# drdh/Homophily-MARL

Measured on NVIDIA B200. Metric: agent-steps/sec (step+obs, device-timed), higher is better.
Workload: dtype u8

## Files before the change

homophily_marl_b200/csrc/ssd_b200.cu:

```cuda
#include <cuda_runtime.h>
#include <stdint.h>
#include <stdlib.h>
#include <string.h>
#include <math.h>
#include <new>
#include <mutex>

#include "ssd_b200.h"

namespace {

constexpr int kWarps = 4;
constexpr int kMinBlocks = 8;
using ColourLuts = uint32_t[kWarps][16];
constexpr uint16_t kNoPoint = 0xFFFF;
constexpr int kMaxDevices = 64;

enum { MODE_STEP = 0, MODE_RESET = 1, MODE_RENDER = 2 };

#ifdef SSD_BOUNDS_CHECK
__device__ unsigned long long g_oob_count = 0;
#define SSD_CHECK(cond) do { if (!(cond)) atomicAdd(&g_oob_count, 1ull); } while (0)
#else
#define SSD_CHECK(cond) do { } while (0)
#endif

struct MapDev {
    uint8_t  base_grid[SSD_MAX_CELLS];
    uint16_t apple_pts[SSD_MAX_CELLS + 4];
    uint16_t waste_pts[SSD_MAX_CELLS + 4];
    uint16_t spawn_pts[SSD_MAX_SPAWN];
    uint32_t thr_apple[SSD_MAX_CELLS + 1];
    uint32_t thr_waste[SSD_MAX_CELLS + 1];
};

struct GeoVals {
    int kind, H, W, V, G, GS, N, RP, PS, AS, LPn, nw8M, nw8T, pitchM, pitchT, PMS;
    int off_map[4];
    int direct, padF, padB;
    uint32_t maskM8;
    int RS4, AS4;
};
__host__ __device__ constexpr int cround_up(int v, int m) { return (v + m - 1) / m * m; }
__host__ __device__ constexpr GeoVals make_geo(int kind, int H, int W, int V) {
    GeoVals g{};
    g.kind = kind; g.H = H; g.W = W; g.V = V; g.G = H * W; g.GS = cround_up(H * W, 16);
    g.N = 2 * V + 1; g.RP = cround_up(g.N, 4); g.PS = g.N * g.RP; g.AS = cround_up(3 * g.PS, 16);
    g.LPn = cround_up(V, 8); g.nw8M = (W + 7) / 8; g.nw8T = (H + 7) / 8;
    g.maskM8 = (W & 7) ? (1u << (4 * (W & 7))) - 1u : 0xffffffffu;
    int wm = (g.LPn + W + V + 7) / 8; if (wm < g.LPn / 8 + g.nw8M) wm = g.LPn / 8 + g.nw8M; if ((wm & 1) == 0) ++wm;
    int wt = (g.LPn + H + V + 7) / 8; if (wt < g.LPn / 8 + g.nw8T) wt = g.LPn / 8 + g.nw8T; if ((wt & 1) == 0) ++wt;
    g.pitchM = 4 * wm; g.pitchT = 4 * wt;
    const int szM = cround_up((H + 2 * V) * g.pitchM, 16) + 16, szT = cround_up((W + 2 * V) * g.pitchT, 16) + 16;
    g.off_map[0] = 16; g.off_map[1] = 16; g.off_map[2] = 16 + szT; g.off_map[3] = 16 + szT;
    g.PMS = szT + szM + 32;
    g.direct = g.RP <= 16;
    g.padF = g.direct ? cround_up(V * W + 48, 16) : 16;
    g.padB = g.direct ? cround_up(V * W + 32, 16) : 32;
    if (g.direct) g.PMS = 0;
    g.RS4 = cround_up((g.N + 1) / 2, 4); g.AS4 = cround_up(g.N * g.RS4, 16);
    return g;
}

struct KParams {
    GeoVals geo;
    int B, n;
    int env0, env1;
    int pdl;
    int NA;
    int agents_uniform;
    int episode_limit, fire_cost, hit_penalty, beam_len, n_actions;
    int n_apple, n_waste, n_spawn, n_apple4, n_waste2;
    int random_spawn, spawn_rot;
    int base_apples, base_waste;
    uint32_t invN20, invW20, invMW20;
    uint32_t seed_lo, seed_hi, gid_base;
    uint32_t thr_harvest[4];
    uint32_t lut[16];
    uint32_t lut8[6];
    const MapDev* map;
    uint8_t* grid; uint32_t* agent; int32_t* ep_ret; int32_t* t; uint32_t* tick; uint32_t* counts;
    const uint8_t* actions; const uint8_t* mask;
    int8_t* reward; uint8_t* clean; uint16_t* apple_cnt; uint8_t* done; uint8_t* obs; uint8_t* state_rgb;
    const uint32_t* d_prio; const uint32_t* d_uapple; const uint32_t* d_uwaste; const uint32_t* d_wkey;
    const uint32_t* d_spawnkey; const uint8_t* d_rot;
    int tag_timeout;
    int state_idx4;
};

template <class D>
struct GeoAccess {
    __device__ __forceinline__ int kind() const { return v().kind; }
    __device__ __forceinline__ int H() const { return v().H; }
    __device__ __forceinline__ int W() const { return v().W; }
    __device__ __forceinline__ int V() const { return v().V; }
    __device__ __forceinline__ int G() const { return v().G; }
    __device__ __forceinline__ int GS() const { return v().GS; }
    __device__ __forceinline__ int N() const { return v().N; }
    __device__ __forceinline__ int RP() const { return v().RP; }
    __device__ __forceinline__ int PS() const { return v().PS; }
    __device__ __forceinline__ int AS() const { return v().AS; }
    __device__ __forceinline__ int RS4() const { return v().RS4; }
    __device__ __forceinline__ int AS4() const { return v().AS4; }
    __device__ __forceinline__ int LPn() const { return v().LPn; }
    __device__ __forceinline__ int nw8M() const { return v().nw8M; }
    __device__ __forceinline__ int nw8T() const { return v().nw8T; }
    __device__ __forceinline__ int pitchM() const { return v().pitchM; }
    __device__ __forceinline__ int pitchT() const { return v().pitchT; }
    __device__ __forceinline__ int PMS() const { return v().PMS; }
    __device__ __forceinline__ bool direct() const { return v().direct != 0; }
    __device__ __forceinline__ int padF() const { return v().padF; }
    __device__ __forceinline__ int padB() const { return v().padB; }
    __device__ __forceinline__ uint32_t maskM8() const { return v().maskM8; }
private:
    __device__ __forceinline__ decltype(auto) v() const { return static_cast<const D*>(this)->vals(); }
};

template <int KIND_, int H_, int W_, int V_>
struct GeoS : GeoAccess<GeoS<KIND_, H_, W_, V_>> {
    static constexpr GeoVals v = make_geo(KIND_, H_, W_, V_);
    __device__ __forceinline__ explicit GeoS(const KParams&) {}
    __device__ __forceinline__ static constexpr GeoVals vals() { return v; }
    __device__ __forceinline__ int off_map(int o) const {
        constexpr int o0 = v.off_map[0], o1 = v.off_map[1], o2 = v.off_map[2], o3 = v.off_map[3];
        return o == 0 ? o0 : (o == 1 ? o1 : (o == 2 ? o2 : o3));
    }
    __device__ __forceinline__ int divW(int x) const { return (int)((unsigned)x / (unsigned)v.W); }
    __device__ __forceinline__ int divN(int x) const { return (int)((unsigned)x / (unsigned)v.N); }
    __device__ __forceinline__ int divMW(int x) const { return (int)((unsigned)x / (unsigned)v.nw8M); }
};

struct GeoD : GeoAccess<GeoD> {
    const KParams& p;
    __device__ __forceinline__ explicit GeoD(const KParams& p_) : p(p_) {}
    __device__ __forceinline__ const GeoVals& vals() const { return p.geo; }
    __device__ __forceinline__ int off_map(int o) const { return p.geo.off_map[o]; }
    __device__ __forceinline__ int divW(int x) const { return (int)(((uint32_t)x * p.invW20) >> 20); }
    __device__ __forceinline__ int divN(int x) const { return (int)(((uint32_t)x * p.invN20) >> 20); }
    __device__ __forceinline__ int divMW(int x) const { return (int)(((uint32_t)x * p.invMW20) >> 20); }
};

__device__ __forceinline__ uint4 philox4x32_10(uint32_t c0, uint32_t c1, uint32_t c2, uint32_t c3,
                                               uint32_t k0, uint32_t k1) {
#pragma unroll
    for (int r = 0; r < 10; ++r) {
        const uint32_t hi0 = __umulhi(0xD2511F53u, c0), lo0 = 0xD2511F53u * c0;
        const uint32_t hi1 = __umulhi(0xCD9E8D57u, c2), lo1 = 0xCD9E8D57u * c2;
        const uint32_t n0 = hi1 ^ c1 ^ k0, n2 = hi0 ^ c3 ^ k1;
        c0 = n0; c1 = lo1; c2 = n2; c3 = lo0;
        k0 += 0x9E3779B9u; k1 += 0xBB67AE85u;
    }
    return make_uint4(c0, c1, c2, c3);
}
__device__ __forceinline__ uint32_t pick(const uint4& v, int i) {
    return i == 0 ? v.x : (i == 1 ? v.y : (i == 2 ? v.z : v.w));
}
struct Warp {
    int lane;
    __device__ __forceinline__ explicit Warp(int lane_) : lane(lane_) {}
    __device__ __forceinline__ unsigned ballot(bool pred) const { return __ballot_sync(0xffffffffu, pred); }
    template <typename T> __device__ __forceinline__ T shfl(T v, int src) const { return __shfl_sync(0xffffffffu, v, src); }
    template <typename T> __device__ __forceinline__ T rmin(T v) const { return __reduce_min_sync(0xffffffffu, v); }
    template <typename T> __device__ __forceinline__ T rmax(T v) const { return __reduce_max_sync(0xffffffffu, v); }
    template <typename T> __device__ __forceinline__ T radd(T v) const { return __reduce_add_sync(0xffffffffu, v); }
    __device__ __forceinline__ unsigned ror(unsigned v) const { return __reduce_or_sync(0xffffffffu, v); }
    __device__ __forceinline__ void sync() const { __syncwarp(); }
};

__device__ __forceinline__ unsigned equal_lanes(const Warp& w, int v, int n) {
    unsigned m = 0;
    for (int j = 0; j < n; ++j) m |= (unsigned)(w.shfl(v, j) == v) << j;
    return m;
}
__device__ __forceinline__ bool surely_distinct(const Warp& w, int v, bool in, unsigned who) {
    const int cnt = __popc(who);
    const unsigned f0 = w.ror(in ? 1u << (v & 31) : 0u);
    if (__popc(f0) == cnt) return true;
    const unsigned f1 = w.ror(in ? 1u << ((v >> 5) & 31) : 0u);
    return __popc(f1) == cnt;
}

template <typename F>
__device__ __forceinline__ void warp_for(int n, int lane, F f) {
    int i = lane;
    if (i < n) f(i);
    for (i += 32; i < n; i += 32) f(i);
}
__device__ __forceinline__ uint32_t philox_word(const KParams& p, uint32_t gid, uint32_t tick, uint32_t stream, uint32_t idx) {
    const uint4 r = philox4x32_10(gid, tick, stream, idx >> 2, p.seed_lo, p.seed_hi);
    return pick(r, idx & 3);
}

__device__ __forceinline__ int agent_colour_index(int i) {
    const int v = i % 10 + 1;
    return 6 + (v == 10 ? 1 : v);
}

template <class GEO>
__device__ __forceinline__ void update_moves(const Warp& w, const GEO& g, const KParams& p, const uint8_t* __restrict__ sg, int lane, bool is_agent,
                                             int act, int& pos, int& ori, int env, uint32_t gid, uint32_t tick) {
    if (act == 5) ori = (0x0132 >> (4 * ori)) & 3;
    else if (act == 6) ori = (0x1023 >> (4 * ori)) & 3;
    const bool mover = is_agent && act <= 4;
    int prop = pos;
    if (mover && act < 4) {
        constexpr uint32_t kDr = (1u) | (1u << 2) | (0u << 4) | (2u << 6) | (1u << 8) | (1u << 10) | (2u << 12) | (0u << 14) |
                                 (0u << 16) | (2u << 18) | (1u << 20) | (1u << 22) | (2u << 24) | (0u << 26) | (1u << 28) | (1u << 30);
        constexpr uint32_t kDc = (2u) | (0u << 2) | (1u << 4) | (1u << 6) | (0u << 8) | (2u << 10) | (1u << 12) | (1u << 14) |
                                 (1u << 16) | (1u << 18) | (0u << 20) | (2u << 22) | (1u << 24) | (1u << 26) | (2u << 28) | (0u << 30);
        const int f = 2 * (ori * 4 + act);
        const int dr = (int)((kDr >> f) & 3u) - 1, dc = (int)((kDc >> f) & 3u) - 1;
        const int q = pos + dr * g.W() + dc;
        SSD_CHECK(q >= 0 && q < g.G());
        prop = sg[q] == SSD_CELL_WALL ? pos : q;
    }
    unsigned in_moves = w.ballot(mover);
    if (in_moves == 0) return;
    int mv = prop;

    unsigned pending = 0;
    if (!surely_distinct(w, prop, mover, in_moves)) {
        const unsigned grp = equal_lanes(w, mover ? prop : -1000 - lane, p.n);
        pending = w.ballot(mover && __popc(grp) >= 2);
    }
    if (pending) {
        uint32_t prio = 0;
        if (mover) prio = p.d_prio ? p.d_prio[(size_t)env * p.n + lane] : philox_word(p, gid, tick, 0, (uint32_t)lane);
        while (pending) {
            const int cell = w.rmin(((pending >> lane) & 1u) ? prop : 0x7fffffff);
            const bool in_cont = mover && prop == cell;
            const unsigned cont = w.ballot(in_cont);
            const unsigned occm = w.ballot(pos == cell);
            bool free_cell = true;
            if (occm) {
                const int occ = 31 - __clz(occm);
                const int mv_occ = w.shfl(mv, occ);
                const bool occ_moves = (in_moves >> occ) & 1u;
                const bool c1 = (cont >> occ) & 1u;
                const bool c2 = !occ_moves || mv_occ == cell;
                const unsigned swp = w.ballot(in_cont && mv_occ == pos);
// ... 608 lines not shown
            d[0] = (uint8_t)rgb; d[g.PS()] = (uint8_t)(rgb >> 8); d[2 * g.PS()] = (uint8_t)(rgb >> 16);
        }
    }
}

template <int MODE, class GEO, bool TAG, bool IDX>
__global__ void __launch_bounds__(kWarps * 32, kMinBlocks) ssd_kernel(const __grid_constant__ KParams p) {
    const GEO g(p);
    extern __shared__ __align__(16) uint8_t smem[];
    __shared__ ColourLuts lut_all;
    const int warp = threadIdx.x >> 5;
    const Warp w(threadIdx.x & 31);
    const int lane = w.lane;
    uint32_t* lut_s = lut_all[warp];
    uint8_t* tile = smem + (size_t)warp * (g.padF() + g.GS() + g.padB() + g.PMS());
    uint8_t* sg = tile + g.padF();
    uint8_t* pmap = sg + g.GS() + g.padB();
    const bool is_agent = lane < p.n;
    const int env = p.env0 + blockIdx.x * kWarps + warp;
    if (env >= p.env1) return;
    auto prologue = [&]() {
        if (lane < 16) lut_s[lane] = p.lut[lane];
        if (p.obs) {
            if (g.direct()) {
                for (int i = lane; i < (g.padF() >> 4); i += 32) reinterpret_cast<uint4*>(tile)[i] = make_uint4(0, 0, 0, 0);
                for (int i = lane; i < (g.padB() >> 4); i += 32) reinterpret_cast<uint4*>(sg + g.GS())[i] = make_uint4(0, 0, 0, 0);
            } else fill_outside(w, g, p, pmap, lane);
        }
    };
    if (p.pdl) {
        prologue();
        asm volatile("griddepcontrol.wait;" ::: "memory");
    }
    {
        if (MODE == MODE_RESET && p.mask && __ldcg(p.mask + env) == 0) return;
        const uint32_t gid = p.gid_base + (uint32_t)env;
        const uint32_t tick = __ldcg(p.tick + env);
        const int t_prev = MODE == MODE_STEP ? __ldcg(p.t + env) : 0;
        const uint32_t cnt = MODE == MODE_STEP ? __ldcg(p.counts + env) : 0u;
        int act = (MODE == MODE_STEP && is_agent) ? (int)__ldcg(p.actions + (size_t)env * p.n + lane) : 255;
        int pos = -1 - lane, ori = 0, ep_ret = 0;
        uint32_t a_rec = 0;
        if (MODE != MODE_RESET && is_agent) {
            a_rec = __ldcg(p.agent + (size_t)env * p.NA + lane);
            ep_ret = __ldcg(p.ep_ret + (size_t)env * p.NA + lane);
        }
        const int n16 = g.GS() >> 4;
        {
            const uint4* src = MODE == MODE_RESET ? reinterpret_cast<const uint4*>(p.map->base_grid)
                                                  : reinterpret_cast<const uint4*>(p.grid + (size_t)env * g.GS());
            uint4 g0 = make_uint4(0, 0, 0, 0);
            if (lane < n16) g0 = __ldcg(src + lane);
            if (!p.pdl) prologue();
            if (lane < n16) reinterpret_cast<uint4*>(sg)[lane] = g0;
            for (int i = lane + 32; i < n16; i += 32) reinterpret_cast<uint4*>(sg)[i] = __ldcg(src + i);
        }
        bool live = is_agent;
        int timer = 0, home = 0;
        if (MODE != MODE_RESET && is_agent) {
            pos = (int)(a_rec & 0xff) * g.W() + (int)((a_rec >> 8) & 0xff);
            ori = (int)((a_rec >> 16) & 3);
            if (TAG) {
                timer = (int)(a_rec >> 24);
                home = pos;
                if (timer) { live = false; pos = -1 - lane; act = 255; }
            }
        }
        w.sync();

        int apples = (int)(cnt & 0xffffu), waste = (int)(cnt >> 16);
        unsigned same = 1u << lane;
        if (MODE == MODE_RENDER) same = equal_lanes(w, pos, p.n);
        if (MODE == MODE_STEP) {
            int reward = 0, clean_num = 0;
            bool tagged = false;
            update_moves(w, g, p, sg, lane, live, act, pos, ori, env, gid, tick);
            same = surely_distinct(w, pos, live, w.ballot(live)) ? (1u << lane) : equal_lanes(w, pos, p.n);
            const int here = live ? sg[pos] : 0;
            const bool first = live && lane == __ffs(same) - 1;
            const unsigned ate = w.ballot(first && here == SSD_CELL_APPLE);
            w.sync();
            if (first) {
                if (here == SSD_CELL_APPLE) { reward += 1; sg[pos] = kOcc | SSD_CELL_EMPTY; }
                else sg[pos] = (uint8_t)(kOcc | here);
            }
            apples -= __popc(ate);
            w.sync();
            beams<TAG>(w, g, p, sg, lane, live, act, pos, ori, reward, clean_num, waste, tagged);
            unsigned gone = 0;
            if (TAG) {
                gone = w.ballot(tagged);
                if (gone) {
                    if (live && lane == __ffs(same) - 1 && (same & ~gone) == 0) sg[pos] &= 0x7f;
                    w.sync();
                    if (tagged) { home = pos; pos = -1 - lane; live = false; }
                }
            }
            spawn(w, g, p, sg, lane, env, gid, tick, apples, waste);
            if (TAG) {
                const bool back = timer == 1;
                timer = tagged ? p.tag_timeout : (timer ? timer - 1 : 0);
                const unsigned who = w.ballot(back);
                if (who) {
                    place_agents<true>(w, g, p, sg, lane, env, gid, tick, who, pos);
                    if (back) { ori = spawn_orientation(p, env, gid, tick, lane); live = true; sg[pos] |= kOcc; }
                    w.sync();
                }
                if (gone | who) same = equal_lanes(w, pos, p.n);
            }
            const int t = t_prev + 1;
            if (is_agent) {
                p.reward[(size_t)env * p.n + lane] = (int8_t)reward;
                p.clean[(size_t)env * p.n + lane] = (uint8_t)clean_num;
                ep_ret += reward;
            }
            if (lane == 0) {
                p.apple_cnt[env] = (uint16_t)apples;
                p.done[env] = t >= p.episode_limit;
                p.t[env] = t;
                p.tick[env] = tick + 1;
                p.counts[env] = (uint32_t)apples | ((uint32_t)waste << 16);
            }
        } else if (MODE == MODE_RESET) {
            place_agents<false>(w, g, p, sg, lane, env, gid, tick, ~0u, pos);
            if (is_agent) ori = spawn_orientation(p, env, gid, tick, lane);
            if (is_agent) sg[pos] |= kOcc;
            w.sync();
            apples = p.base_apples; waste = p.base_waste;
            spawn(w, g, p, sg, lane, env, gid, tick, apples, waste);
            ep_ret = 0;
            if (lane == 0) { p.t[env] = 0; p.tick[env] = tick + 1; p.counts[env] = (uint32_t)apples | ((uint32_t)waste << 16); }
        }

        if (p.pdl) asm volatile("griddepcontrol.launch_dependents;" ::: "memory");
        if (MODE != MODE_RENDER) {
            if (live && lane == __ffs(same) - 1) sg[pos] &= 0x7f;
            w.sync();
            uint4* dst = reinterpret_cast<uint4*>(p.grid + (size_t)env * g.GS());
            warp_for(g.GS() >> 4, lane, [&](int i) { dst[i] = reinterpret_cast<const uint4*>(sg)[i]; });
            if (is_agent) {
                const int cell = (TAG && !live) ? home : pos;
                const int r = g.divW(cell);
                p.agent[(size_t)env * p.NA + lane] = (uint32_t)r | ((uint32_t)(cell - r * g.W()) << 8) | ((uint32_t)ori << 16)
                                                     | (TAG ? (uint32_t)timer << 24 : 0u);
                p.ep_ret[(size_t)env * p.NA + lane] = ep_ret;
            }
        }
        if (p.obs || p.state_rgb) {
            w.sync();
            if (IDX) { if (live && lane == 31 - __clz(same)) sg[pos] = (uint8_t)(p.agents_uniform ? 7 : agent_colour_index(lane)); }
            else if (live) sg[pos] = 7;
            w.sync();
            const unsigned outm = TAG ? w.ballot(is_agent && !live) : 0u;
            render<IDX>(w, g, p, sg, pmap, lut_s, lane, is_agent, live, pos, ori, env, same, outm);
        }
    }
}

__global__ void incentive_kernel(const long long* __restrict__ a_inc, const float* __restrict__ reward, long long rows, int n,
                                 float incentive, float cost, float ratio, float T, int recip,
                                 float* __restrict__ r_env, float* __restrict__ r_inc, float* __restrict__ sgn) {
    const long long idx = (long long)blockIdx.x * blockDim.x + threadIdx.x;
    if (idx >= rows * n) return;
    const long long row = idx / n;
    const int k = (int)(idx - row * n);
    const long long* a = a_inc + row * n * n;
    int give = 0, rp = 0, rn = 0;
    for (int j = 0; j < n; ++j) {
        if (j == k) continue;
        give += a[k * n + j] != 0;
        const long long v = a[j * n + k];
        rp += v == 1; rn += v == 2;
    }
    const float rv = (float)(rp - rn), r = reward[idx];
    const float e = __fadd_rn(r, __fmul_rn(__fmul_rn(rv, ratio), incentive));
    const float c = __fsub_rn(r, __fmul_rn(__fmul_rn((float)give, cost), incentive));
    if (recip) { const float inv = __fdiv_rn(1.0f, T); r_env[idx] = __fmul_rn(e, inv); r_inc[idx] = __fmul_rn(c, inv); }
    else { r_env[idx] = __fdiv_rn(e, T); r_inc[idx] = __fdiv_rn(c, T); }
    if (sgn) sgn[idx] = rv > 0.f ? 1.f : (rv < 0.f ? -1.f : 0.f);
}

struct ExpandParams {
    const uint8_t* in;
    float* out;
    int rows, cols, row_stride, block_stride;
    uint32_t lut[16];
};
__global__ void __launch_bounds__(256) expand_index4_kernel(const __grid_constant__ ExpandParams p) {
    const uint8_t* __restrict__ in = p.in + (size_t)blockIdx.x * p.block_stride;
    const int NN = p.rows * p.cols;
    float* __restrict__ out = p.out + (size_t)blockIdx.x * 3 * NN;
    for (int q = threadIdx.x; q < NN; q += blockDim.x) {
        const int y = q / p.cols, x = q - y * p.cols;
        const uint32_t rgb = p.lut[(__ldg(in + y * p.row_stride + (x >> 1)) >> (4 * (x & 1))) & 15u];
        out[q] = (float)(rgb & 0xffu) * (1.0f / 256.0f);
        out[NN + q] = (float)((rgb >> 8) & 0xffu) * (1.0f / 256.0f);
        out[2 * NN + q] = (float)((rgb >> 16) & 0xffu) * (1.0f / 256.0f);
    }
}

thread_local int g_last_cuda_error = 0;

inline int cuda_fail(cudaError_t e) { g_last_cuda_error = (int)e; return SSD_ERR_CUDA; }
#define SSD_CUDA(x) do { cudaError_t e_ = (x); if (e_ != cudaSuccess) return cuda_fail(e_); } while (0)

inline int round_up(int v, int m) { return (v + m - 1) / m * m; }

struct DeviceGuard {
    int prev = -1;
    bool switched = false;
    cudaError_t err = cudaSuccess;
    explicit DeviceGuard(int dev) {
        err = cudaGetDevice(&prev);
        if (err == cudaSuccess && prev != dev) { err = cudaSetDevice(dev); switched = err == cudaSuccess; }
    }
    ~DeviceGuard() { if (switched) cudaSetDevice(prev); }
};

uint32_t magic20(int d, int max_x) {
    uint32_t m = (uint32_t)(((1u << 20) + d - 1) / d);
    for (int x = 0; x <= max_x; ++x)
        if ((int)(((uint64_t)x * m) >> 20) != x / d) return 0;
    return m;
}

ssd_obs_layout obs_layout(const KParams& k, int32_t format) {
    const GeoVals& g = k.geo;
    if (format == SSD_OBS_INDEX4) return { format, g.RS4, 0, g.AS4, k.n * g.AS4 };
    return { format, g.RP, g.PS, g.AS, k.n * g.AS };
}

ssd_state_layout state_layout(const KParams& k, int32_t format) {
    const GeoVals& g = k.geo;
    if (format == SSD_OBS_INDEX4) return { format, 4 * g.nw8M, 0, 4 * round_up(g.H * g.nw8M, 4) };
    return { format, g.W, g.G, 3 * g.G };
}

}

struct ssd_handle {
    KParams kp;
    MapDev* d_map;
    int device;
    size_t smem_bytes;
    mutable int64_t launches;
    int force_generic;
    int pdl;
    int obs_format;
    int state_format;
};

static int fill_common(const ssd_handle* h, const ssd_state* st, const ssd_draws* d, KParams& k) {
    if (!h || !st || !st->grid || !st->agent || !st->ep_ret || !st->t || !st->tick || !st->counts) return SSD_ERR_INVALID;
    k = h->kp;
    k.env0 = 0; k.env1 = k.B;
    k.state_idx4 = h->state_format == SSD_OBS_INDEX4;
    k.grid = st->grid; k.agent = st->agent; k.ep_ret = st->ep_ret; k.t = st->t; k.tick = st->tick; k.counts = st->counts;
    if (d) {
        if ((d->u_waste == nullptr) != (d->wkey == nullptr)) return SSD_ERR_INVALID;
        k.d_prio = d->prio; k.d_uapple = d->u_apple; k.d_uwaste = d->u_waste; k.d_wkey = d->wkey;
        k.d_spawnkey = d->spawn_key; k.d_rot = d->rot;
    }
    return SSD_OK;
}

template <int MODE, class GEO, bool TAG, bool IDX>
static int launch_kernel(ssd_handle* h, const KParams& k, void* stream) {
    DeviceGuard guard(h->device);
    SSD_CUDA(guard.err);
    {
        static std::mutex mu;
        static int high_water[kMaxDevices] = {};
        std::lock_guard<std::mutex> lock(mu);
        const int dev = h->device;
        if (dev < 0 || dev >= kMaxDevices) return SSD_ERR_INVALID;
        if ((int)h->smem_bytes > high_water[dev]) {
            SSD_CUDA(cudaFuncSetAttribute(ssd_kernel<MODE, GEO, TAG, IDX>, cudaFuncAttributeMaxDynamicSharedMemorySize, (int)h->smem_bytes));
            high_water[dev] = (int)h->smem_bytes;
        }
    }
    const int grid = (k.env1 - k.env0 + kWarps - 1) / kWarps;
    if (grid <= 0) return SSD_OK;

    if (k.pdl) {
        cudaLaunchConfig_t cfg = {};
        cfg.gridDim = dim3((unsigned)grid); cfg.blockDim = dim3(kWarps * 32); cfg.dynamicSmemBytes = h->smem_bytes;
        cfg.stream = (cudaStream_t)stream;
        cudaLaunchAttribute attr[1];
        attr[0].id = cudaLaunchAttributeProgrammaticStreamSerialization;
        attr[0].val.programmaticStreamSerializationAllowed = 1;
        cfg.attrs = attr; cfg.numAttrs = 1;
        SSD_CUDA(cudaLaunchKernelEx(&cfg, ssd_kernel<MODE, GEO, TAG, IDX>, k));
    } else {
        ssd_kernel<MODE, GEO, TAG, IDX><<<grid, kWarps * 32, h->smem_bytes, (cudaStream_t)stream>>>(k);
    }
    ++h->launches;
    SSD_CUDA(cudaGetLastError());
    return SSD_OK;
}

constexpr int kPdlMaxEnvs = 2048;

template <int MODE, class GEO>
static int launch_geo(ssd_handle* h, const KParams& k_in, void* stream) {
    KParams k = k_in;
    k.pdl = h->pdl && (k.env1 - k.env0) <= kPdlMaxEnvs;
    const bool idx = h->obs_format == SSD_OBS_INDEX4;
    if constexpr (MODE != MODE_RESET) {
        if (k.tag_timeout != 0)
            return idx ? launch_kernel<MODE, GEO, true, true>(h, k, stream) : launch_kernel<MODE, GEO, true, false>(h, k, stream);
    }
    return idx ? launch_kernel<MODE, GEO, false, true>(h, k, stream) : launch_kernel<MODE, GEO, false, false>(h, k, stream);
}

template <int MODE>
static int launch(ssd_handle* h, const KParams& k, void* stream) {
    const GeoVals& v = k.geo;
    if (!h->force_generic) {
        if (v.kind == SSD_KIND_HARVEST && v.H == 9 && v.W == 38 && v.V == 15) return launch_geo<MODE, GeoS<SSD_KIND_HARVEST, 9, 38, 15>>(h, k, stream);
        if (v.kind == SSD_KIND_HARVEST && v.H == 9 && v.W == 38 && v.V == 7) return launch_geo<MODE, GeoS<SSD_KIND_HARVEST, 9, 38, 7>>(h, k, stream);
        if (v.kind == SSD_KIND_CLEANUP && v.H == 25 && v.W == 18 && v.V == 7) return launch_geo<MODE, GeoS<SSD_KIND_CLEANUP, 25, 18, 7>>(h, k, stream);
        if (v.kind == SSD_KIND_CLEANUP && v.H == 48 && v.W == 18 && v.V == 7) return launch_geo<MODE, GeoS<SSD_KIND_CLEANUP, 48, 18, 7>>(h, k, stream);
        if (v.kind == SSD_KIND_CLEANUP && v.H == 10 && v.W == 10 && v.V == 7) return launch_geo<MODE, GeoS<SSD_KIND_CLEANUP, 10, 10, 7>>(h, k, stream);
    }
    return launch_geo<MODE, GeoD>(h, k, stream);
}

extern "C" {

int ssd_abi_version(void) { return SSD_B200_ABI_VERSION; }

const char* ssd_error_string(int code) {
    switch (code) {
        case SSD_OK: return "ok";
        case SSD_ERR_INVALID: return "invalid argument or unsupported geometry";
        case SSD_ERR_CUDA: return "CUDA runtime error";
        case SSD_ERR_SPAWN: return "There are not enough spawn points! Check your map?";
        case SSD_ERR_MAP: return "map must be wall-enclosed and use the reference alphabet";
        default: return "unknown error";
    }
}

int ssd_last_cuda_error(void) { return g_last_cuda_error; }

uint32_t ssd_prob_to_threshold(double p) {
    if (!(p > 0.0)) return 0u;
    const double t = ceil(p * 4294967296.0);
    return t >= 4294967295.0 ? 0xFFFFFFFFu : (uint32_t)t;
}

int ssd_create(const ssd_config* cfg, ssd_handle** out) {
    if (!cfg || !out || !cfg->ascii_map) return SSD_ERR_INVALID;
    *out = nullptr;
    const int H = cfg->height, W = cfg->width, G = H * W, n = cfg->n_agents, V = cfg->view;
    if (cfg->kind != SSD_KIND_CLEANUP && cfg->kind != SSD_KIND_HARVEST) return SSD_ERR_INVALID;
    if (H < 3 || W < 3 || H > 255 || W > 255 || G > SSD_MAX_CELLS) return SSD_ERR_INVALID;
    if (n < 1 || n > SSD_MAX_AGENTS || V < 1 || V > 31 || cfg->n_envs < 1) return SSD_ERR_INVALID;
    if (cfg->beam_len < 0 || cfg->episode_limit < 1 || cfg->spawn_rotation > 3) return SSD_ERR_INVALID;
    if (abs(cfg->fire_cost) + n * abs(cfg->hit_penalty) + 1 > 127) return SSD_ERR_INVALID;
    if (cfg->tag_timeout < 0 || cfg->tag_timeout > 255) return SSD_ERR_INVALID;

    MapDev* hm = new (std::nothrow) MapDev;
    if (!hm) return SSD_ERR_INVALID;
    memset(hm, 0, sizeof(MapDev));
    int na = 0, nw = 0, ns = 0;
    for (int c = 0; c < G; ++c) {
        const char ch = cfg->ascii_map[c];
        const int r = c / W, col = c % W;
        const bool border = r == 0 || col == 0 || r == H - 1 || col == W - 1;
        if (border && ch != '@') { delete hm; return SSD_ERR_MAP; }
        uint8_t code = SSD_CELL_EMPTY;
        switch (ch) {
            case '@': code = SSD_CELL_WALL; break;
            case ' ': break;
            case 'P': if (ns < SSD_MAX_SPAWN) hm->spawn_pts[ns] = (uint16_t)c; ++ns; break;
            case 'A': if (cfg->kind == SSD_KIND_HARVEST) { code = SSD_CELL_APPLE; hm->apple_pts[na++] = (uint16_t)c; } break;
            case 'B': if (cfg->kind == SSD_KIND_CLEANUP) hm->apple_pts[na++] = (uint16_t)c; break;
            case 'H': if (cfg->kind == SSD_KIND_CLEANUP) { code = SSD_CELL_WASTE; hm->waste_pts[nw++] = (uint16_t)c; } break;
            case 'R': if (cfg->kind == SSD_KIND_CLEANUP) code = SSD_CELL_RIVER; break;
            case 'S': if (cfg->kind == SSD_KIND_CLEANUP) code = SSD_CELL_STREAM; break;
            default: delete hm; return SSD_ERR_MAP;
        }
        hm->base_grid[c] = code;
    }
    if (ns < n) { delete hm; return SSD_ERR_SPAWN; }
    if (ns > SSD_MAX_SPAWN) { delete hm; return SSD_ERR_INVALID; }
    for (int k = na; k < round_up(na, 4) + 4 && k < SSD_MAX_CELLS + 4; ++k) hm->apple_pts[k] = kNoPoint;
    for (int k = nw; k < round_up(nw, 2) + 2 && k < SSD_MAX_CELLS + 4; ++k) hm->waste_pts[k] = kNoPoint;
    if (cfg->kind == SSD_KIND_CLEANUP) {
        if (cfg->n_waste_lut != (uint32_t)nw + 1 || !cfg->thr_apple || !cfg->thr_waste) { delete hm; return SSD_ERR_INVALID; }
        memcpy(hm->thr_apple, cfg->thr_apple, sizeof(uint32_t) * (nw + 1));
        memcpy(hm->thr_waste, cfg->thr_waste, sizeof(uint32_t) * (nw + 1));
    }

    ssd_handle* h = new (std::nothrow) ssd_handle;
    if (!h) { delete hm; return SSD_ERR_INVALID; }
    memset(h, 0, sizeof(*h));
    KParams& k = h->kp;
    k.geo = make_geo(cfg->kind, H, W, V);
    const GeoVals& gv = k.geo;
    k.B = cfg->n_envs; k.n = n; k.NA = round_up(n, 4);
    k.episode_limit = cfg->episode_limit; k.fire_cost = cfg->fire_cost; k.hit_penalty = cfg->hit_penalty;
    k.tag_timeout = cfg->tag_timeout;
    k.beam_len = cfg->beam_len; k.n_actions = cfg->kind == SSD_KIND_CLEANUP ? 9 : 8;
    k.n_apple = na; k.n_waste = nw; k.n_spawn = ns; k.n_apple4 = (na + 3) / 4; k.n_waste2 = (nw + 1) / 2;
    k.base_apples = 0; k.base_waste = 0;
    for (int c = 0; c < G; ++c) { k.base_apples += hm->base_grid[c] == SSD_CELL_APPLE; k.base_waste += hm->base_grid[c] == SSD_CELL_WASTE; }
    k.random_spawn = cfg->random_spawn_point != 0; k.spawn_rot = cfg->spawn_rotation < 0 ? -1 : cfg->spawn_rotation;
    k.invN20 = magic20(gv.N, SSD_MAX_AGENTS * gv.N + 64); k.invW20 = magic20(W, G + 1);
    k.seed_lo = (uint32_t)cfg->seed; k.seed_hi = (uint32_t)(cfg->seed >> 32); k.gid_base = cfg->env_gid_base;
    for (int i = 0; i < 4; ++i) k.thr_harvest[i] = cfg->thr_harvest[i];
    for (int i = 0; i < 16; ++i)
        k.lut[i] = (uint32_t)cfg->color_lut[i][0] | ((uint32_t)cfg->color_lut[i][1] << 8) | ((uint32_t)cfg->color_lut[i][2] << 16);
    k.agents_uniform = 1;
    for (int i = 8; i < 16; ++i) if (k.lut[i] != k.lut[7]) k.agents_uniform = 0;
    for (int ch = 0; ch < 3; ++ch) {
        uint32_t lo = 0, hi = 0;
        for (int i = 0; i < 4; ++i) { lo |= (uint32_t)cfg->color_lut[i][ch] << (8 * i); hi |= (uint32_t)cfg->color_lut[4 + i][ch] << (8 * i); }
        k.lut8[2 * ch] = lo; k.lut8[2 * ch + 1] = hi;
    }
    if (k.invN20 == 0 || k.invW20 == 0 || k.n_apple4 > 32 * 16) { delete hm; delete h; return SSD_ERR_INVALID; }

    k.invMW20 = magic20(gv.nw8M, H * gv.nw8M + 32);
    if (k.invMW20 == 0 || gv.PMS >= 60000) { delete hm; delete h; return SSD_ERR_INVALID; }
    h->smem_bytes = (size_t)kWarps * (gv.padF + gv.GS + gv.padB + gv.PMS);
    { const char* e = getenv("SSD_B200_GENERIC"); h->force_generic = e && e[0] == '1'; }
    { const char* e = getenv("SSD_B200_PDL"); h->pdl = !(e && e[0] == '0'); }
    h->device = cfg->device;

    DeviceGuard guard(cfg->device);
    cudaError_t e = guard.err;
    if (e == cudaSuccess) {
        int optin = 0;
        e = cudaDeviceGetAttribute(&optin, cudaDevAttrMaxSharedMemoryPerBlockOptin, cfg->device);
        if (e == cudaSuccess && h->smem_bytes + sizeof(ColourLuts) > (size_t)optin) { delete hm; delete h; return SSD_ERR_INVALID; }
    }
    if (e == cudaSuccess) e = cudaMalloc(&h->d_map, sizeof(MapDev));
    if (e == cudaSuccess) e = cudaMemcpy(h->d_map, hm, sizeof(MapDev), cudaMemcpyHostToDevice);
    delete hm;
    if (e != cudaSuccess) {
        if (h->d_map) cudaFree(h->d_map);
        delete h;
        return cuda_fail(e);
    }
    k.map = h->d_map;
    *out = h;
    return SSD_OK;
}

int ssd_destroy(ssd_handle* h) {
    if (!h) return SSD_ERR_INVALID;
    DeviceGuard guard(h->device);
    cudaFree(h->d_map);
    delete h;
    return SSD_OK;
}

int ssd_get_layout(const ssd_handle* h, ssd_layout* o) {
    if (!h || !o) return SSD_ERR_INVALID;
    const KParams& k = h->kp;
    const GeoVals& g = k.geo;
    o->n_actions = k.n_actions; o->n_cells = g.G; o->obs_n = g.N; o->grid_stride = g.GS; o->agent_stride = k.NA;
    o->obs_plane_stride = g.PS; o->obs_agent_stride = g.AS; o->obs_env_stride = obs_layout(k, SSD_OBS_RGB).env_stride;
    o->n_apple_pts = k.n_apple; o->n_waste_pts = k.n_waste; o->n_spawn_pts = k.n_spawn; o->obs_row_stride = g.RP;
    return SSD_OK;
}

int ssd_get_obs_layout(const ssd_handle* h, int32_t format, ssd_obs_layout* o) {
    if (!h || !o || (format != SSD_OBS_RGB && format != SSD_OBS_INDEX4)) return SSD_ERR_INVALID;
    *o = obs_layout(h->kp, format);
    return SSD_OK;
}

int ssd_set_obs_format(ssd_handle* h, int32_t format) {
    if (!h || (format != SSD_OBS_RGB && format != SSD_OBS_INDEX4)) return SSD_ERR_INVALID;
    h->obs_format = format;
    return SSD_OK;
}

int ssd_get_state_layout(const ssd_handle* h, int32_t format, ssd_state_layout* o) {
    if (!h || !o || (format != SSD_OBS_RGB && format != SSD_OBS_INDEX4)) return SSD_ERR_INVALID;
    *o = state_layout(h->kp, format);
    return SSD_OK;
}

int ssd_set_state_format(ssd_handle* h, int32_t format) {
    if (!h || (format != SSD_OBS_RGB && format != SSD_OBS_INDEX4)) return SSD_ERR_INVALID;
    h->state_format = format;
    return SSD_OK;
}

int ssd_reset(ssd_handle* h, const ssd_state* st, const uint8_t* mask, const ssd_draws* draws, uint8_t* obs, void* stream) {
    KParams k;
    const int rc = fill_common(h, st, draws, k);
    if (rc) return rc;
    k.mask = mask; k.obs = obs;
    return launch<MODE_RESET>(h, k, stream);
}

int ssd_step(ssd_handle* h, const ssd_state* st, const uint8_t* actions, const ssd_draws* draws,
             const ssd_step_out* out, void* stream) {
    return ssd_step_range(h, st, actions, draws, out, 0, h ? h->kp.B : 0, stream);
}

int ssd_step_range(ssd_handle* h, const ssd_state* st, const uint8_t* actions, const ssd_draws* draws,
                   const ssd_step_out* out, int32_t env_begin, int32_t env_count, void* stream) {
    KParams k;
    const int rc = fill_common(h, st, draws, k);
    if (rc) return rc;
    if (!actions || !out || !out->reward || !out->clean || !out->apple_cnt || !out->done) return SSD_ERR_INVALID;
    if (env_begin < 0 || env_count < 0 || (int64_t)env_begin + env_count > k.B) return SSD_ERR_INVALID;
    k.env0 = env_begin; k.env1 = env_begin + env_count;
    k.actions = actions; k.reward = out->reward; k.clean = out->clean; k.apple_cnt = out->apple_cnt; k.done = out->done;
    k.obs = out->obs; k.state_rgb = out->state_rgb;
    return launch<MODE_STEP>(h, k, stream);
}

int ssd_render(ssd_handle* h, const ssd_state* st, uint8_t* obs, uint8_t* state_rgb, void* stream) {
    KParams k;
    const int rc = fill_common(h, st, nullptr, k);
    if (rc) return rc;
    if (!obs && !state_rgb) return SSD_ERR_INVALID;
    k.obs = obs; k.state_rgb = state_rgb;
    return launch<MODE_RENDER>(h, k, stream);
}

int ssd_step_host(ssd_handle* h, const ssd_state* st, const uint8_t* h_actions, uint8_t* d_actions,
                  const ssd_step_out* d_out, const ssd_step_out* h_out, void* stream) {
    if (!h || !h_actions || !d_actions || !d_out || !h_out) return SSD_ERR_INVALID;
    DeviceGuard guard(h->device);
    SSD_CUDA(guard.err);
    const KParams& k = h->kp;
    cudaStream_t s = (cudaStream_t)stream;
    const size_t B = (size_t)k.B;
    SSD_CUDA(cudaMemcpyAsync(d_actions, h_actions, B * k.n, cudaMemcpyHostToDevice, s));
    const int rc = ssd_step(h, st, d_actions, nullptr, d_out, stream);
    if (rc) return rc;
    if (h_out->reward) SSD_CUDA(cudaMemcpyAsync(h_out->reward, d_out->reward, B * k.n, cudaMemcpyDeviceToHost, s));
    if (h_out->clean) SSD_CUDA(cudaMemcpyAsync(h_out->clean, d_out->clean, B * k.n, cudaMemcpyDeviceToHost, s));
    if (h_out->apple_cnt) SSD_CUDA(cudaMemcpyAsync(h_out->apple_cnt, d_out->apple_cnt, B * 2, cudaMemcpyDeviceToHost, s));
    if (h_out->done) SSD_CUDA(cudaMemcpyAsync(h_out->done, d_out->done, B, cudaMemcpyDeviceToHost, s));
    const size_t ES = (size_t)obs_layout(k, h->obs_format).env_stride;
    if (h_out->obs && d_out->obs) SSD_CUDA(cudaMemcpyAsync(h_out->obs, d_out->obs, B * ES, cudaMemcpyDeviceToHost, s));
    if (h_out->state_rgb && d_out->state_rgb)
        SSD_CUDA(cudaMemcpyAsync(h_out->state_rgb, d_out->state_rgb, B * (size_t)state_layout(k, h->state_format).env_stride,
                                 cudaMemcpyDeviceToHost, s));
    SSD_CUDA(cudaStreamSynchronize(s));
    return SSD_OK;
}

int ssd_incentive(const int64_t* actions_inc, const float* reward, int64_t rows, int32_t n_agents,
                  float incentive, float cost, float ratio, int32_t max_seq_length,
                  float* rewards_for_env, float* rewards_for_inc, float* recv_sign, void* stream) {
    if (!actions_inc || !reward || !rewards_for_env || !rewards_for_inc || rows < 0 || n_agents < 1 || max_seq_length == 0)
        return SSD_ERR_INVALID;
    if (rows == 0) return SSD_OK;
    const int recip = max_seq_length < 0;
    const float T = (float)abs(max_seq_length);
    const long long total = (long long)rows * n_agents;
    const int threads = 256;
    incentive_kernel<<<(unsigned)((total + threads - 1) / threads), threads, 0, (cudaStream_t)stream>>>(
        reinterpret_cast<const long long*>(actions_inc), reward, rows, n_agents, incentive, cost, ratio, T, recip,
        rewards_for_env, rewards_for_inc, recv_sign);
    SSD_CUDA(cudaGetLastError());
    return SSD_OK;
}

static int launch_expand(const ssd_handle* h, const uint8_t* in, int64_t blocks, int rows, int cols, int row_stride,
                         int block_stride, float* out, void* stream) {
    DeviceGuard guard(h->device);
    SSD_CUDA(guard.err);
    ExpandParams e;
    e.in = in; e.out = out;
    e.rows = rows; e.cols = cols; e.row_stride = row_stride; e.block_stride = block_stride;
    for (int i = 0; i < 16; ++i) e.lut[i] = h->kp.lut[i];
    expand_index4_kernel<<<(unsigned)blocks, 256, 0, (cudaStream_t)stream>>>(e);
    ++h->launches;
    SSD_CUDA(cudaGetLastError());
    return SSD_OK;
}

int ssd_expand_obs(const ssd_handle* h, const uint8_t* obs_index4, int32_t env_begin, int32_t env_count, float* out, void* stream) {
    if (!h || !obs_index4 || !out) return SSD_ERR_INVALID;
    const KParams& k = h->kp;
    if (env_begin < 0 || env_count < 0 || (int64_t)env_begin + env_count > k.B) return SSD_ERR_INVALID;
    if (env_count == 0) return SSD_OK;
    const GeoVals& g = k.geo;
    return launch_expand(h, obs_index4 + (size_t)env_begin * k.n * g.AS4, (int64_t)env_count * k.n, g.N, g.N, g.RS4, g.AS4,
                         out, stream);
}

int ssd_expand_state(const ssd_handle* h, const uint8_t* state_index4, int32_t env_begin, int32_t env_count, float* out,
                     void* stream) {
    if (!h || !state_index4 || !out) return SSD_ERR_INVALID;
    const KParams& k = h->kp;
    if (env_begin < 0 || env_count < 0 || (int64_t)env_begin + env_count > k.B) return SSD_ERR_INVALID;
    if (env_count == 0) return SSD_OK;
    const ssd_state_layout s = state_layout(k, SSD_OBS_INDEX4);
    return launch_expand(h, state_index4 + (size_t)env_begin * s.env_stride, env_count, k.geo.H, k.geo.W, s.row_stride,
                         s.env_stride, out, stream);
}

int64_t ssd_launch_count(const ssd_handle* h) { return h ? h->launches : -1; }

int64_t ssd_debug_oob_count(void) {
#ifdef SSD_BOUNDS_CHECK
    unsigned long long v = 0;
    if (cudaDeviceSynchronize() != cudaSuccess || cudaMemcpyFromSymbol(&v, g_oob_count, sizeof(v)) != cudaSuccess) return -2;
    return (int64_t)v;
#else
    return -1;
#endif
}

}
```

Before: 1.912 billion.

## Split RGB step into index4 render plus separate LUT expand kernel for ranges

For ranged steps with RGB obs on 32-wide-row geometries, the step kernel now renders compact 4-bit index observations into a scratch buffer, records the per-env out-of-play agent mask, and then launches a separate expand kernel. That kernel converts index rows into RGB planes with byte-permute lookups. The intent is to take the wide RGB writes off the warp-per-env step kernel and do them in a fully parallel bandwidth-bound pass. The cost is an extra launch and a scratch-buffer round trip through memory. A microbenchmark probe is also added.

```diff
diff --git a/homophily_marl_b200/csrc/ssd_b200.cu b/homophily_marl_b200/csrc/ssd_b200.cu
--- a/homophily_marl_b200/csrc/ssd_b200.cu
+++ b/homophily_marl_b200/csrc/ssd_b200.cu
@@ -86,6 +86,7 @@
     const uint32_t* d_spawnkey; const uint8_t* d_rot;
     int tag_timeout;
     int state_idx4;
+    uint32_t* outm;
 };
 
 template <class D>
@@ -1000,6 +1001,7 @@
             else if (live) sg[pos] = 7;
             w.sync();
             const unsigned outm = TAG ? w.ballot(is_agent && !live) : 0u;
+            if (TAG && p.outm && lane == 0) p.outm[env] = outm;
             render<IDX>(w, g, p, sg, pmap, lut_s, lane, is_agent, live, pos, ori, env, same, outm);
         }
     }
@@ -1047,6 +1049,60 @@
     }
 }
 
+struct RgbExpandParams {
+    const uint8_t* idx;
+    const uint32_t* outm;
+    uint8_t* obs;
+    int rows, N, n, AS4, AS, PS;
+    uint32_t lastmask;
+    uint32_t lut[3][4];
+    int pdl;
+};
+template <int RP, bool FULL>
+__global__ void __launch_bounds__(512) expand_rgb_kernel(const __grid_constant__ RgbExpandParams p) {
+    if (p.pdl) {
+        asm volatile("griddepcontrol.launch_dependents;" ::: "memory");
+        asm volatile("griddepcontrol.wait;" ::: "memory");
+    }
+    constexpr int WR = RP / 4;
+    for (int u = blockIdx.x * blockDim.x + threadIdx.x; u < p.rows; u += gridDim.x * blockDim.x) {
+        const int v = (unsigned)u / (unsigned)p.N, y = u - v * p.N;
+        uint32_t s[WR / 2];
+        if constexpr (RP == 32) {
+            const uint4 q = __ldg(reinterpret_cast<const uint4*>(p.idx + (size_t)v * p.AS4 + y * (RP / 2)));
+            s[0] = q.x; s[1] = q.y; s[2] = q.z; s[3] = q.w;
+        } else {
+            const uint2 q = __ldg(reinterpret_cast<const uint2*>(p.idx + (size_t)v * p.AS4 + y * (RP / 2)));
+            s[0] = q.x; s[1] = q.y;
+        }
+        uint32_t keep = 0xffffffffu;
+        if (p.outm) {
+            const int e = (unsigned)v / (unsigned)p.n;
+            keep = ((__ldg(p.outm + e) >> (v - e * p.n)) & 1u) ? 0u : 0xffffffffu;
+        }
+        uint8_t* dst = p.obs + (size_t)v * p.AS + y * RP;
+#pragma unroll
+        for (int pl = 0; pl < 3; ++pl) {
+            uint32_t o[WR];
+#pragma unroll
+            for (int k = 0; k < WR; ++k) {
+                const uint32_t sel = s[k >> 1] >> (16 * (k & 1));
+                if constexpr (FULL) {
+                    const uint32_t lo = prmt(p.lut[pl][0], p.lut[pl][1], sel & 0x7777u);
+                    const uint32_t hi = prmt(p.lut[pl][2], p.lut[pl][3], sel & 0x7777u);
+                    const uint32_t m = prmt(0u, 0xffffffffu, (sel >> 1) & 0x4444u);
+                    o[k] = ((lo & ~m) | (hi & m)) & keep;
+                } else {
+                    o[k] = prmt(p.lut[pl][0], p.lut[pl][1], sel) & keep;
+                }
+            }
+            o[WR - 1] &= p.lastmask;
+            if constexpr (RP == 32) st_row32(dst + pl * p.PS, o);
+            else st_row16(dst + pl * p.PS, o);
+        }
+    }
+}
+
 thread_local int g_last_cuda_error = 0;
 
 inline int cuda_fail(cudaError_t e) { g_last_cuda_error = (int)e; return SSD_ERR_CUDA; }
@@ -1096,6 +1152,8 @@
     int pdl;
     int obs_format;
     int state_format;
+    int split_rgb;
+    uint8_t* d_split;
 };
 
 static int fill_common(const ssd_handle* h, const ssd_state* st, const ssd_draws* d, KParams& k) {
@@ -1150,10 +1208,9 @@
 constexpr int kPdlMaxEnvs = 2048;
 
 template <int MODE, class GEO>
-static int launch_geo(ssd_handle* h, const KParams& k_in, void* stream) {
+static int launch_geo(ssd_handle* h, const KParams& k_in, bool idx, void* stream) {
     KParams k = k_in;
     k.pdl = h->pdl && (k.env1 - k.env0) <= kPdlMaxEnvs;
-    const bool idx = h->obs_format == SSD_OBS_INDEX4;
     if constexpr (MODE != MODE_RESET) {
         if (k.tag_timeout != 0)
             return idx ? launch_kernel<MODE, GEO, true, true>(h, k, stream) : launch_kernel<MODE, GEO, true, false>(h, k, stream);
@@ -1162,16 +1219,66 @@
 }
 
 template <int MODE>
-static int launch(ssd_handle* h, const KParams& k, void* stream) {
+static int launch(ssd_handle* h, const KParams& k, void* stream, bool idx) {
     const GeoVals& v = k.geo;
     if (!h->force_generic) {
-        if (v.kind == SSD_KIND_HARVEST && v.H == 9 && v.W == 38 && v.V == 15) return launch_geo<MODE, GeoS<SSD_KIND_HARVEST, 9, 38, 15>>(h, k, stream);
-        if (v.kind == SSD_KIND_HARVEST && v.H == 9 && v.W == 38 && v.V == 7) return launch_geo<MODE, GeoS<SSD_KIND_HARVEST, 9, 38, 7>>(h, k, stream);
-        if (v.kind == SSD_KIND_CLEANUP && v.H == 25 && v.W == 18 && v.V == 7) return launch_geo<MODE, GeoS<SSD_KIND_CLEANUP, 25, 18, 7>>(h, k, stream);
-        if (v.kind == SSD_KIND_CLEANUP && v.H == 48 && v.W == 18 && v.V == 7) return launch_geo<MODE, GeoS<SSD_KIND_CLEANUP, 48, 18, 7>>(h, k, stream);
-        if (v.kind == SSD_KIND_CLEANUP && v.H == 10 && v.W == 10 && v.V == 7) return launch_geo<MODE, GeoS<SSD_KIND_CLEANUP, 10, 10, 7>>(h, k, stream);
-    }
-    return launch_geo<MODE, GeoD>(h, k, stream);
+        if (v.kind == SSD_KIND_HARVEST && v.H == 9 && v.W == 38 && v.V == 15) return launch_geo<MODE, GeoS<SSD_KIND_HARVEST, 9, 38, 15>>(h, k, idx, stream);
+        if (v.kind == SSD_KIND_HARVEST && v.H == 9 && v.W == 38 && v.V == 7) return launch_geo<MODE, GeoS<SSD_KIND_HARVEST, 9, 38, 7>>(h, k, idx, stream);
+        if (v.kind == SSD_KIND_CLEANUP && v.H == 25 && v.W == 18 && v.V == 7) return launch_geo<MODE, GeoS<SSD_KIND_CLEANUP, 25, 18, 7>>(h, k, idx, stream);
+        if (v.kind == SSD_KIND_CLEANUP && v.H == 48 && v.W == 18 && v.V == 7) return launch_geo<MODE, GeoS<SSD_KIND_CLEANUP, 48, 18, 7>>(h, k, idx, stream);
+        if (v.kind == SSD_KIND_CLEANUP && v.H == 10 && v.W == 10 && v.V == 7) return launch_geo<MODE, GeoS<SSD_KIND_CLEANUP, 10, 10, 7>>(h, k, idx, stream);
+    }
+    return launch_geo<MODE, GeoD>(h, k, idx, stream);
+}
+template <int MODE>
+static int launch(ssd_handle* h, const KParams& k, void* stream) { return launch<MODE>(h, k, stream, h->obs_format == SSD_OBS_INDEX4); }
+
+constexpr int kSplitMaxEnvs = kPdlMaxEnvs;
+constexpr int kExpandThreads = 256;
+
+static bool split_geometry(const GeoVals& g) { return g.RP == 32; }
+static size_t split_bytes(const KParams& k) { return (size_t)k.B * (k.n * k.geo.AS4 + 4); }
+
+static int launch_expand_rgb(ssd_handle* h, const KParams& k, uint8_t* obs, void* stream) {
+    DeviceGuard guard(h->device);
+    SSD_CUDA(guard.err);
+    const GeoVals& g = k.geo;
+    const size_t idx_bytes = (size_t)k.B * k.n * g.AS4;
+    RgbExpandParams e;
+    e.idx = h->d_split + (size_t)k.env0 * k.n * g.AS4;
+    e.outm = k.tag_timeout != 0 ? reinterpret_cast<const uint32_t*>(h->d_split + idx_bytes) + k.env0 : nullptr;
+    e.obs = obs + (size_t)k.env0 * k.n * g.AS;
+    e.rows = (k.env1 - k.env0) * k.n * g.N;
+    e.N = g.N; e.n = k.n; e.AS4 = g.AS4; e.AS = g.AS; e.PS = g.PS;
+    e.lastmask = 0xffffffffu >> (8 * (g.RP - g.N));
+    for (int pl = 0; pl < 3; ++pl)
+        for (int w = 0; w < 4; ++w) {
+            uint32_t v = 0;
+            for (int b = 0; b < 4; ++b) v |= ((k.lut[4 * w + b] >> (8 * pl)) & 0xffu) << (8 * b);
+            e.lut[pl][w] = v;
+        }
+    e.pdl = h->pdl;
+    const void* fn = k.agents_uniform ? (const void*)expand_rgb_kernel<32, false> : (const void*)expand_rgb_kernel<32, true>;
+    cudaLaunchConfig_t cfg = {};
+    cfg.gridDim = dim3((unsigned)((e.rows + kExpandThreads - 1) / kExpandThreads)); cfg.blockDim = dim3(kExpandThreads);
+    cfg.stream = (cudaStream_t)stream;
+    cudaLaunchAttribute attr[1];
+    attr[0].id = cudaLaunchAttributeProgrammaticStreamSerialization;
+    attr[0].val.programmaticStreamSerializationAllowed = 1;
+    cfg.attrs = attr; cfg.numAttrs = e.pdl ? 1 : 0;
+    void* args[] = { &e };
+    SSD_CUDA(cudaLaunchKernelExC(&cfg, fn, args));
+    ++h->launches;
+    SSD_CUDA(cudaGetLastError());
+    return SSD_OK;
+}
+
+static int set_split_scratch(ssd_handle* h, bool rgb) {
+    DeviceGuard guard(h->device);
+    SSD_CUDA(guard.err);
+    if (rgb && h->split_rgb && !h->d_split) SSD_CUDA(cudaMalloc(&h->d_split, split_bytes(h->kp)));
+    if (!rgb && h->d_split) { SSD_CUDA(cudaFree(h->d_split)); h->d_split = nullptr; }
+    return SSD_OK;
 }
 
 extern "C" {
@@ -1292,6 +1399,9 @@
         return cuda_fail(e);
     }
     k.map = h->d_map;
+    { const char* e = getenv("SSD_B200_SPLIT_RGB"); h->split_rgb = !(e && e[0] == '0') && split_geometry(gv); }
+    const int rc = set_split_scratch(h, true);
+    if (rc) { cudaFree(h->d_map); delete h; return rc; }
     *out = h;
     return SSD_OK;
 }
@@ -1300,6 +1410,7 @@
     if (!h) return SSD_ERR_INVALID;
     DeviceGuard guard(h->device);
     cudaFree(h->d_map);
+    cudaFree(h->d_split);
     delete h;
     return SSD_OK;
 }
@@ -1322,6 +1433,8 @@
 
 int ssd_set_obs_format(ssd_handle* h, int32_t format) {
     if (!h || (format != SSD_OBS_RGB && format != SSD_OBS_INDEX4)) return SSD_ERR_INVALID;
+    const int rc = set_split_scratch(h, format == SSD_OBS_RGB);
+    if (rc) return rc;
     h->obs_format = format;
     return SSD_OK;
 }
@@ -1346,13 +1459,8 @@
     return launch<MODE_RESET>(h, k, stream);
 }
 
-int ssd_step(ssd_handle* h, const ssd_state* st, const uint8_t* actions, const ssd_draws* draws,
-             const ssd_step_out* out, void* stream) {
-    return ssd_step_range(h, st, actions, draws, out, 0, h ? h->kp.B : 0, stream);
-}
-
-int ssd_step_range(ssd_handle* h, const ssd_state* st, const uint8_t* actions, const ssd_draws* draws,
-                   const ssd_step_out* out, int32_t env_begin, int32_t env_count, void* stream) {
+static int step_impl(ssd_handle* h, const ssd_state* st, const uint8_t* actions, const ssd_draws* draws,
+                     const ssd_step_out* out, int32_t env_begin, int32_t env_count, bool ranges, void* stream) {
     KParams k;
     const int rc = fill_common(h, st, draws, k);
     if (rc) return rc;
@@ -1361,7 +1469,23 @@
     k.env0 = env_begin; k.env1 = env_begin + env_count;
     k.actions = actions; k.reward = out->reward; k.clean = out->clean; k.apple_cnt = out->apple_cnt; k.done = out->done;
     k.obs = out->obs; k.state_rgb = out->state_rgb;
+    if (ranges && out->obs && h->d_split && env_count > 0 && env_count <= kSplitMaxEnvs) {
+        k.obs = h->d_split;
+        k.outm = reinterpret_cast<uint32_t*>(h->d_split + (size_t)k.B * k.n * k.geo.AS4);
+        const int rc2 = launch<MODE_STEP>(h, k, stream, true);
+        return rc2 ? rc2 : launch_expand_rgb(h, k, out->obs, stream);
+    }
     return launch<MODE_STEP>(h, k, stream);
+}
+
+int ssd_step(ssd_handle* h, const ssd_state* st, const uint8_t* actions, const ssd_draws* draws,
+             const ssd_step_out* out, void* stream) {
+    return step_impl(h, st, actions, draws, out, 0, h ? h->kp.B : 0, false, stream);
+}
+
+int ssd_step_range(ssd_handle* h, const ssd_state* st, const uint8_t* actions, const ssd_draws* draws,
+                   const ssd_step_out* out, int32_t env_begin, int32_t env_count, void* stream) {
+    return step_impl(h, st, actions, draws, out, env_begin, env_count, true, stream);
 }
 
 int ssd_render(ssd_handle* h, const ssd_state* st, uint8_t* obs, uint8_t* state_rgb, void* stream) {
diff --git a/profiles/microbench/rgb_expand_probe.cu b/profiles/microbench/rgb_expand_probe.cu
--- /dev/null
+++ b/profiles/microbench/rgb_expand_probe.cu
@@ -0,0 +1,100 @@
+#include "../../homophily_marl_b200/csrc/ssd_b200.cu"
+
+#include <algorithm>
+#include <cstdio>
+#include <vector>
+
+namespace {
+
+constexpr int kEnvs = 4096, kRanges = 8, kN = 5, kV = 15, kRing = 4, kSteps = 200, kReplays = 7;
+
+#define CK(x) do { cudaError_t e_ = (x); if (e_ != cudaSuccess) { fprintf(stderr, "%s: %s\n", #x, cudaGetErrorString(e_)); exit(1); } } while (0)
+
+struct Probe {
+    GeoVals g = make_geo(SSD_KIND_HARVEST, 9, 38, kV);
+    uint8_t* idx = nullptr;
+    uint8_t* ring[kRing] = {};
+    size_t env_rgb = 0, env_idx = 0;
+    cudaStream_t main_s, rs[kRanges];
+    cudaEvent_t fork, join[kRanges];
+
+    RgbExpandParams params(int env0, int envs, int t) const {
+        RgbExpandParams e{};
+        e.idx = idx + env0 * env_idx; e.outm = nullptr; e.obs = ring[t % kRing] + env0 * env_rgb;
+        e.rows = envs * kN * g.N; e.N = g.N; e.n = kN; e.AS4 = g.AS4; e.AS = g.AS; e.PS = g.PS;
+        e.lastmask = 0xffffffffu >> (8 * (g.RP - g.N));
+        for (int pl = 0; pl < 3; ++pl) for (int w = 0; w < 4; ++w) e.lut[pl][w] = 0x40302010u * (pl + 1) + 0x04040404u * w;
+        e.pdl = 0;
+        return e;
+    }
+    void launch(const RgbExpandParams& e, int threads, int rpt, cudaStream_t s) const {
+        const int grid = (e.rows + threads * rpt - 1) / (threads * rpt);
+        expand_rgb_kernel<32, false><<<grid, threads, 0, s>>>(e);
+    }
+    cudaGraph_t capture(bool ranges, int threads, int rpt) {
+        cudaGraph_t gr;
+        CK(cudaStreamBeginCapture(main_s, cudaStreamCaptureModeThreadLocal));
+        if (ranges) {
+            CK(cudaEventRecord(fork, main_s));
+            for (int r = 0; r < kRanges; ++r) {
+                CK(cudaStreamWaitEvent(rs[r], fork, 0));
+                for (int t = 0; t < kSteps; ++t) launch(params(r * (kEnvs / kRanges), kEnvs / kRanges, t), threads, rpt, rs[r]);
+                CK(cudaEventRecord(join[r], rs[r]));
+                CK(cudaStreamWaitEvent(main_s, join[r], 0));
+            }
+        } else {
+            for (int t = 0; t < kSteps; ++t) launch(params(0, kEnvs, t), threads, rpt, main_s);
+        }
+        CK(cudaStreamEndCapture(main_s, &gr));
+        return gr;
+    }
+    void time(const char* what, bool ranges, int threads, int rpt) {
+        cudaGraph_t gr = capture(ranges, threads, rpt);
+        cudaGraphExec_t ex;
+        CK(cudaGraphInstantiate(&ex, gr, 0));
+        cudaEvent_t e0, e1;
+        CK(cudaEventCreate(&e0)); CK(cudaEventCreate(&e1));
+        CK(cudaGraphLaunch(ex, main_s));
+        std::vector<float> us;
+        for (int i = 0; i < kReplays; ++i) {
+            CK(cudaEventRecord(e0, main_s));
+            CK(cudaGraphLaunch(ex, main_s));
+            CK(cudaEventRecord(e1, main_s));
+            CK(cudaEventSynchronize(e1));
+            float ms = 0;
+            CK(cudaEventElapsedTime(&ms, e0, e1));
+            us.push_back(ms * 1000.f / kSteps);
+        }
+        std::sort(us.begin(), us.end());
+        const double bytes = (double)kEnvs * env_rgb;
+        printf("{\"arrangement\": \"%s\", \"threads\": %d, \"rows_per_thread\": %d, \"us_per_step\": %.3f, \"us_min\": %.3f, "
+               "\"us_max\": %.3f, \"rgb_TBps\": %.3f}\n", what, threads, rpt, us[kReplays / 2], us[0], us[kReplays - 1],
+               bytes / (us[kReplays / 2] * 1e-6) / 1e12);
+        fflush(stdout);
+        CK(cudaEventDestroy(e0)); CK(cudaEventDestroy(e1));
+        CK(cudaGraphExecDestroy(ex)); CK(cudaGraphDestroy(gr));
+    }
+};
+
+}
+
+int main() {
+    Probe P;
+    P.env_rgb = (size_t)kN * P.g.AS; P.env_idx = (size_t)kN * P.g.AS4;
+    CK(cudaMalloc(&P.idx, kEnvs * P.env_idx));
+    std::vector<uint8_t> h(kEnvs * P.env_idx);
+    uint32_t x = 12345u;
+    for (auto& b : h) { x = x * 1664525u + 1013904223u; b = (uint8_t)((x >> 24) & 0x77u); }
+    CK(cudaMemcpy(P.idx, h.data(), h.size(), cudaMemcpyHostToDevice));
+    for (auto& r : P.ring) CK(cudaMalloc(&r, kEnvs * P.env_rgb));
+    CK(cudaStreamCreateWithFlags(&P.main_s, cudaStreamNonBlocking));
+    for (auto& s : P.rs) CK(cudaStreamCreateWithFlags(&s, cudaStreamNonBlocking));
+    CK(cudaEventCreateWithFlags(&P.fork, cudaEventDisableTiming));
+    for (auto& e : P.join) CK(cudaEventCreateWithFlags(&e, cudaEventDisableTiming));
+    for (int threads : {128, 256, 512})
+        for (int rpt : {1, 2, 4}) {
+            P.time("ranges8", true, threads, rpt);
+            P.time("one4096", false, threads, rpt);
+        }
+    return 0;
+}
diff --git a/profiles/rgb_expand_probe.py b/profiles/rgb_expand_probe.py
--- /dev/null
+++ b/profiles/rgb_expand_probe.py
@@ -0,0 +1,38 @@
+from __future__ import annotations
+
+import argparse
+import json
+import os
+import subprocess
+import sys
+import tempfile
+
+HERE = os.path.dirname(os.path.abspath(__file__))
+ROOT = os.path.dirname(HERE)
+sys.path.insert(0, ROOT)
+
+
+def main():
+    ap = argparse.ArgumentParser()
+    ap.add_argument("--out", default=None)
+    a = ap.parse_args()
+    from homophily_marl_b200._build import nvcc_path
+    lines = []
+    q = subprocess.run(["nvidia-smi", "--query-gpu=name,power.limit,clocks.max.sm", "--format=csv,noheader"],
+                       capture_output=True, text=True)
+    lines.append(json.dumps({"gpu": q.stdout.strip()}))
+    with tempfile.TemporaryDirectory() as td:
+        exe = os.path.join(td, "rgb_expand_probe")
+        subprocess.run([nvcc_path(), "-O3", "-std=c++17", "-gencode", "arch=compute_100a,code=sm_100a",
+                        "-I", os.path.join(ROOT, "include"), "-o", exe, os.path.join(HERE, "microbench", "rgb_expand_probe.cu")],
+                       check=True)
+        r = subprocess.run([exe], capture_output=True, text=True, check=True)
+    lines += [ln for ln in r.stdout.splitlines() if ln.strip()]
+    print("\n".join(lines))
+    if a.out:
+        with open(a.out, "w") as f:
+            f.write("\n".join(lines) + "\n")
+
+
+if __name__ == "__main__":
+    main()
```

New measurement: 1.339 billion, median of 6. -30.0%, worse.
